# rongmon/rbvfit

Measured on AMD Instinct MI355X. Metric: walker-lnprob evals/sec, higher is better.
Workload: dtype f64; 1 GPU; C1: MgII 2796/2803 z=0.348, 2 components, 4096 px, 23-tap Gaussian LSF; walkers_per_gpu=512, walkers_total=512, ndim=6, n_lines=4, parallelism=walker-shard x1

## Files before the change

rbvfit_amd/csrc/capi_context.inc:

```
namespace {

thread_local std::string g_create_error;
#ifdef VP_STAMPS
double g_host_stamps[8];
std::chrono::steady_clock::time_point g_host_t0;
#define VP_HSTAMP(k) g_host_stamps[k] = std::chrono::duration<double, std::nano>(std::chrono::steady_clock::now() - g_host_t0).count()
#else
#define VP_HSTAMP(k) do { } while (0)
#endif

struct Tuning {
    int prep_rpw = 64;
    int geom = -1;
    int finalize = -1;
    int walker = -1;
    long zerocopy_max = 1l << 20;
    int no_zerocopy = 0;
    int no_multipole = 0;
    int multipole_min = 3;
    int span = 0;
    int waves = 0;
    long lds_pad = 0;
    int no_fused_accept = 0;
    int farfield = -1;
    int no_shared_prep = 0;
    int walker_clusters = 0;
    int multi_sync = 0;
    int host_spin = 2;
    int no_ff_members = 0;
    int tile_multi = -1;
    int gather_plain = 0;
    int tile_lpt = 1;
    int slice_rows = 2;
    int flux_farfield = -1;
    int walker_prio = -1;
    long walker_perm_hex = 0;
    int walker_perm = -1;
    int stretch_overlap = -1;
    int prearm = -1;
    int prearm_us = 500;
    int flux_walker = 1;
    int stretch_mailbox = 1;
    int walker_split = 0;
    int slice_seg = 0;
};

struct Knob { const char* name; const char* env; int is_long; size_t off; };
#define VP_KNOB(field, envname, is_long) {#field, envname, is_long, offsetof(Tuning, field)}
const Knob g_knobs[] = {
    VP_KNOB(prep_rpw, "RBVFIT_AMD_PREP_RPW", 0), VP_KNOB(geom, "RBVFIT_AMD_GEOM", 0),
    VP_KNOB(finalize, "RBVFIT_AMD_FINALIZE", 0), VP_KNOB(walker, "RBVFIT_AMD_WALKER", 0),
    VP_KNOB(zerocopy_max, "RBVFIT_AMD_ZEROCOPY_MAX", 1),
    VP_KNOB(no_zerocopy, "RBVFIT_AMD_NO_ZEROCOPY", 0), VP_KNOB(no_multipole, "RBVFIT_AMD_NO_MULTIPOLE", 0), VP_KNOB(multipole_min, "RBVFIT_AMD_MULTIPOLE_MIN", 0),
    VP_KNOB(span, "RBVFIT_AMD_SPAN", 0), VP_KNOB(waves, "RBVFIT_AMD_WAVES", 0), VP_KNOB(lds_pad, "RBVFIT_AMD_LDS_PAD", 1),
    VP_KNOB(no_fused_accept, "RBVFIT_AMD_NO_FUSED_ACCEPT", 0), VP_KNOB(slice_rows, "RBVFIT_AMD_SLICE_ROWS", 0), VP_KNOB(walker_clusters, "RBVFIT_AMD_WALKER_CLUSTERS", 0), VP_KNOB(no_shared_prep, "RBVFIT_AMD_NO_SHARED_PREP", 0),
    VP_KNOB(farfield, "RBVFIT_AMD_FARFIELD", 0), VP_KNOB(multi_sync, "RBVFIT_AMD_MULTI_SYNC", 0), VP_KNOB(tile_multi, "RBVFIT_AMD_TILE_MULTI", 0), VP_KNOB(no_ff_members, "RBVFIT_AMD_NO_FF_MEMBERS", 0), VP_KNOB(host_spin, "RBVFIT_AMD_HOST_SPIN", 0),
    VP_KNOB(tile_lpt, "RBVFIT_AMD_TILE_LPT", 0), VP_KNOB(gather_plain, "RBVFIT_AMD_GATHER_PLAIN", 0), VP_KNOB(slice_seg, "RBVFIT_AMD_SLICE_SEG", 0),
    VP_KNOB(flux_farfield, "RBVFIT_AMD_FLUX_FARFIELD", 0), VP_KNOB(stretch_overlap, "RBVFIT_AMD_STRETCH_OVERLAP", 0), VP_KNOB(stretch_mailbox, "RBVFIT_AMD_STRETCH_MAILBOX", 0), VP_KNOB(flux_walker, "RBVFIT_AMD_FLUX_WALKER", 0), VP_KNOB(walker_perm, "RBVFIT_AMD_WALKER_PERM", 0), VP_KNOB(walker_prio, "RBVFIT_AMD_WALKER_PRIO", 0), VP_KNOB(walker_perm_hex, "RBVFIT_AMD_WALKER_PERM_HEX", 1),
    VP_KNOB(prearm, "RBVFIT_AMD_PREARM", 0), VP_KNOB(prearm_us, "RBVFIT_AMD_PREARM_US", 0), VP_KNOB(walker_split, "RBVFIT_AMD_WALKER_SPLIT", 0),
};
void set_knob(Tuning& t, const Knob& k, long v) {
    char* base = reinterpret_cast<char*>(&t) + k.off;
    if (k.is_long) *reinterpret_cast<long*>(base) = v; else *reinterpret_cast<int*>(base) = (int)v;
}
Tuning tuning_from_env() {
    Tuning t;
    for (const Knob& k : g_knobs)
        if (const char* e = getenv(k.env))
            set_knob(t, k, *e ? (std::strcmp(k.name, "walker_perm_hex") == 0 ? (long)strtoull(e, nullptr, 16) : strtol(e, nullptr, 10)) : 1);
    return t;
}

struct Instrument {
    vp::InstDev dev{};
    vp::InstDev dev_s{};
    vp::InstDev dev_w{};
    size_t lds_w = 0;
    size_t lds_s = 0;
    int* split_hint = nullptr;
    unsigned long long wperm = 0xFEDCBA9876543210ull;
    unsigned long long wperm_shared = 0xFEDCBA9876543210ull;
    int deal_ntask = 0;
    std::vector<long> deal_cost;

    vp::LinesDev lines{};
    double sum_logw = 0.0;
    std::vector<void*> allocs;
    double* d_flux = nullptr;
    double* d_w = nullptr;
    size_t lds_bytes = 0;
    std::vector<double> h_lambda0, h_gamma;
    std::vector<int> h_bidx;
    bool needs_generic = true;
    bool nanfix = false;
    int nwaves = 1;
    bool ff_on = false;
    double ff_cover = 0.0;
    int ff_items = 0;
    std::vector<double> h_lines;
    std::vector<int> h_idx;
    unsigned long long member_mask[2] = {0ull, 0ull};
    bool same_lines_as_prev = false;
    int* fisher_off = nullptr;
    int2* fisher_terms = nullptr;
// ... 130 lines not shown
int fail(const vp_ctx* c, int code, const std::string& msg) {
    if (c) c->err = msg; else g_create_error = msg;
    return code;
}

#define HIP_TRY(c, expr)                                                                     \
    do {                                                                                     \
        hipError_t e__ = (expr);                                                             \
        if (e__ != hipSuccess)                                                               \
            return fail((c), VP_EHIP, std::string(#expr) + ": " + hipGetErrorString(e__));   \
    } while (0)

template <class T>
int upload(vp_ctx* c, Instrument* ins, const T* host, size_t n, T** out, size_t pad = 0) {
    T* d = nullptr;
    HIP_TRY(c, hipMalloc((void**)&d, ((n ? n : 1) + pad) * sizeof(T)));
    if (ins) ins->allocs.push_back(d);
    if (pad) HIP_TRY(c, hipMemset(d + n, 0, pad * sizeof(T)));
    if (n) HIP_TRY(c, hipMemcpy(d, host, n * sizeof(T), hipMemcpyHostToDevice));
    *out = d;
    return VP_OK;
}

double neumaier_sum(const double* v, int n) {
    double s = 0.0, comp = 0.0;
    for (int i = 0; i < n; ++i) {
        double t = s + v[i];
        if (std::fabs(s) >= std::fabs(v[i])) comp += (s - t) + v[i]; else comp += (v[i] - t) + s;
        s = t;
    }
    return s + comp;
}

constexpr uint64_t VP_SENTINEL_BITS = 0x7FF8A5C3965A3C69ull;
inline bool carries_sentinel(const double* v, size_t n) {
    bool hit = false;
    for (size_t i = 0; i < n; ++i) {
        uint64_t b;
        std::memcpy(&b, v + i, 8);
        hit |= ((b & 0x7FFFFFFFFFFFFFFFull) | 0x0008000000000000ull) == VP_SENTINEL_BITS;
    }
    return hit;
}

int ensure_scratch(vp_ctx* c, size_t bytes) {
    if (bytes <= c->scratch_bytes) return VP_OK;
// ... 93 lines not shown
```

rbvfit_amd/csrc/capi_launch.inc:

```
struct TileOpts {
    const vp::InstDev* geom = nullptr;
    int grid_z = 1;
    double* ff = nullptr;
    int gen_slots = 0;
    const double* theta_rebuild = nullptr;
    int D = 0;
};
template <int OUT, bool GENERIC>
void launch_tile(const Instrument& in, const double* lc, const int* flags, double* out, int stride, int offset,
                 int W, hipStream_t s, const vp::FinalizeArgs& fin, const int* genflag, const TileOpts& o = TileOpts{}) {
    const vp::InstDev& dev = o.geom ? *o.geom : in.dev;
    const bool fast = dev.method == VP_VOIGT_FAST;
    dim3 grid(W, dev.ntiles, o.grid_z);
    dim3 block(64 * in.nwaves);
    const dim3 gg(o.gen_slots > 0 ? std::min(W, o.gen_slots) : W, dev.ntiles, o.grid_z);
    if (dev.rbot && OUT != 2) {
        constexpr int O = OUT == 1 ? 1 : 0;
        if (GENERIC)
            hipLaunchKernelGGL((vp::tile_generic_kernel<O, false, true>), gg, block, in.lds_bytes, s, dev, lc, flags, out, stride, offset, fin, genflag, W,
                               in.lines, (const double*)nullptr, 0);
        else
            hipLaunchKernelGGL((fast ? vp::tile_kernel<1, O, false, false, true> : vp::tile_kernel<0, O, false, false, true>), grid, block, in.lds_bytes, s,
                               dev, lc, flags, out, stride, offset, fin, genflag);
        return;
// ... 190 lines not shown
        if (c->inst.size() == 2)
            hipLaunchKernelGGL((fast ? vp::walker_kernel2<1, SAMPLER, ARMED> : vp::walker_kernel2<0, SAMPLER, ARMED>), grid, block, lds, s, dk[0], dk[1], tb, t0, a, st);
        else
            hipLaunchKernelGGL((fast ? vp::walker_kernel4<1, SAMPLER, ARMED> : vp::walker_kernel4<0, SAMPLER, ARMED>), grid, block, lds, s, dk[0], dk[1], dk[2], dk[3],
                               tb, t0, a, st);
        return;
    }
    hipLaunchKernelGGL((fast ? vp::walker_kernel<1, false, SAMPLER, ARMED> : keep_clusters ? vp::walker_kernel<0, true, false, ARMED>
                                                                                            : vp::walker_kernel<0, false, SAMPLER, ARMED>),
                       grid, block, lds, s, d0, t0, a, st);
}

unsigned long long walker_deal_for(vp_ctx* c, int W, bool shared_ok) {
    const unsigned long long ident = 0xFEDCBA9876543210ull;
    const int mode = c->tune.walker_perm;
    if (c->inst.size() != 1 || mode == 0) return ident;
    if (c->tune.walker_perm_hex != 0) return (unsigned long long)c->tune.walker_perm_hex;
    const Instrument& in = c->inst[0];
    if (mode == 1) return in.wperm;
    if (mode == 2 && shared_ok) return in.wperm_shared;
    if (ctx_num_cus(c) > 0 && W <= ctx_num_cus(c)) return in.wperm;
    return shared_ok ? in.wperm_shared : ident;
}
int walker_prio_for(vp_ctx* c, int W) {
    if (c->tune.walker_prio >= 0) return c->tune.walker_prio ? 1 : 0;
    return (ctx_num_cus(c) > 0 && W <= ctx_num_cus(c)) ? 0 : 1;
}

vp::WalkerArgs walker_args(vp_ctx* c, int W, const double* theta, double* out, double sum_logw, int split = 0, int row0 = 0,
                           bool shared_cus = false, bool shared_ok = false) {
    const Instrument& in = c->inst[0];
    const size_t nrec = (size_t)(in.dev.L + in.dev.NCm) * vp::LC_STRIDE;
    const int per = std::max(1, split);
    vp::WalkerArgs a{theta, c->d_lb, c->d_ub, c->d_lc + (size_t)row0 * per * nrec, out, sum_logw, c->D,
                     (int)((split > 0 ? in.lds_s : walker_wave_lds(c)) / sizeof(double)),
                     (shared_cus && c->tune.walker_prio < 0) ? 1 : walker_prio_for(c, W * per),
                     split > 0 ? 0xFEDCBA9876543210ull : walker_deal_for(c, W, shared_ok)};
    if (split > 0) { a.split = split; a.split_row0 = row0; a.split_part = c->d_partial; a.split_ticket = c->d_ticket; }
    return a;
}

struct LaunchPlan {
    int kind = 0;
    int split = 0;
    int Wp = 0;
    int sel = 0;
    int fmode = 0;
    int ff_first = -1;
    int ff_first_blk = 0;
};
const vp::InstDev& geom_of(const Instrument& x, int sel) { return sel == 2 ? x.dev_w : sel ? x.dev_s : x.dev; }

void launch_walker(vp_ctx* c, const LaunchPlan& p, int W, const double* d_theta, double* d_out, hipStream_t s, bool armed = false) {
    vp::WalkerArgs a = walker_args(c, W, d_theta, d_out, c->inst[0].sum_logw, p.split, 0, false, !armed);
    if (armed) {
        a.arm_slots = c->arm.slots;
        a.arm_slot_doubles = c->arm.slot_doubles;
        a.arm_host = c->arm.h_dev;
        a.arm_seq = c->arm.seq;
        const int cap = std::min(std::max(1, c->tune.prearm_us), 100000);
// ... 213 lines not shown
```

rbvfit_amd/csrc/capi_misc.inc:

```
void vp_philox4x32(const uint32_t ctr[4], const uint32_t key[2], uint32_t out[4]) {
    const vp::Philox4 r = vp::philox4x32_10(ctr[0], ctr[1], ctr[2], ctr[3], key[0], key[1]);
    for (int i = 0; i < 4; ++i) out[i] = r.v[i];
}

int vp_voigt_h(vp_ctx* c, int na, const double* a, int nx, const double* x, double* out) {
    if (!c) return VP_EINVAL;
    CtxGuard g(c);
    if (na <= 0 || nx <= 0 || !a || !x || !out) return fail(c, VP_EINVAL, "vp_voigt_h: empty or NULL input");
    HIP_TRY(c, hipSetDevice(c->device));
    const size_t rec = (size_t)na * vp::LC_STRIDE, need = (rec + na + nx + (size_t)na * nx) * sizeof(double);
    int rc;
    if ((rc = ensure_scratch(c, need))) return rc;
    double* d_rec = c->d_scratch;
    double* d_a = d_rec + rec;
    double* d_x = d_a + na;
    double* d_o = d_x + nx;
    HIP_TRY(c, hipMemcpyAsync(d_a, a, na * sizeof(double), hipMemcpyHostToDevice, c->stream));
    HIP_TRY(c, hipMemcpyAsync(d_x, x, nx * sizeof(double), hipMemcpyHostToDevice, c->stream));
    hipLaunchKernelGGL(vp::prep_h_kernel, dim3((na + 63) / 64), dim3(64), 0, c->stream, d_a, (int)na, d_rec);
    hipLaunchKernelGGL(vp::voigt_h_kernel, dim3((nx + 255) / 256, na), dim3(256), 0, c->stream, d_rec, d_x, nx, d_o);
    HIP_TRY(c, hipGetLastError());
    HIP_TRY(c, hipMemcpyAsync(out, d_o, (size_t)na * nx * sizeof(double), hipMemcpyDeviceToHost, c->stream));
    HIP_TRY(c, hipStreamSynchronize(c->stream));
    return VP_OK;
// ... 58 lines not shown
    if (pairs) *pairs = 0;
    const vp_ctx::LastFF lf = c->last_ff;
    if (lf.inst < 0 || !lf.ff || lf.W <= 0 || lf.nbk <= 0) return VP_OK;
    HIP_TRY(c, hipSetDevice(c->device));
    HIP_TRY(c, hipDeviceSynchronize());
    const size_t n = (size_t)lf.W * lf.nbk;
    std::vector<double> h(n * vp::FF_STRIDE);
    HIP_TRY(c, hipMemcpy(h.data(), lf.ff, h.size() * sizeof(double), hipMemcpyDeviceToHost));
    const Instrument& in = c->inst[lf.inst];
    int64_t cov = 0, mem = 0;
    for (size_t i = 0; i < n; ++i) {
        unsigned long long m[2];
        memcpy(m, h.data() + i * vp::FF_STRIDE + vp::FF_MASK0, sizeof m);
        cov += __builtin_popcountll(m[0]) + __builtin_popcountll(m[1]);
        mem += __builtin_popcountll(m[0] & in.member_mask[0]) + __builtin_popcountll(m[1] & in.member_mask[1]);
    }
    if (variant) *variant = lf.members ? 2 : 1;
    if (covered) *covered = cov;
    if (covered_members) *covered_members = mem;
    if (pairs) *pairs = (int64_t)n * in.lines.L;
    return VP_OK;
}

int vp_walker_deals(const vp_ctx* c, int inst, uint64_t deals[2], int64_t* cost, int max_tiles, int* ntiles, int* ntask) {
    if (!c) return VP_EINVAL;
    std::lock_guard<std::mutex> g(c->mu);
    if (inst < 0 || inst >= (int)c->inst.size()) return VP_EINVAL;
    const Instrument& in = c->inst[inst];
    if (deals) { deals[0] = in.wperm; deals[1] = in.wperm_shared; }
    if (ntiles) *ntiles = in.dev_w.ntiles;
    if (ntask) *ntask = in.deal_ntask;
    for (int t = 0; cost && t < max_tiles; ++t) cost[t] = t < (int)in.deal_cost.size() ? in.deal_cost[t] : 0;
    return VP_OK;
}
int vp_last_launch_kind(const vp_ctx* c) {
    if (!c) return -1;
    std::lock_guard<std::mutex> g(c->mu);
    return c->last_kind;
}
int vp_last_walker_split(const vp_ctx* c) {
    if (!c) return -1;
    std::lock_guard<std::mutex> g(c->mu);
    return c->last_kind == 1 ? c->last_split : 0;
}
```

rbvfit_amd/csrc/capi_setup.inc:

```

const char* vp_version(void) { return "rbvfit_amd " RBVFIT_AMD_VERSION " (gfx950, hip)"; }

int vp_device_count(void) {
    int n = 0;
    if (hipGetDeviceCount(&n) != hipSuccess) return 0;
    return n;
}

const char* vp_last_error(const vp_ctx* ctx) { return ctx ? ctx->err.c_str() : g_create_error.c_str(); }

int vp_ctx_create(vp_ctx** out, int device_id) {
    if (!out) return fail(nullptr, VP_EINVAL, "out is NULL");
    *out = nullptr;
    int n = 0;
    hipError_t e = hipGetDeviceCount(&n);
    if (e != hipSuccess || n <= 0)
        return fail(nullptr, VP_EHIP, std::string("no usable HIP device: ") + (e != hipSuccess ? hipGetErrorString(e) : "device count is 0"));
    if (device_id < 0 || device_id >= n) return fail(nullptr, VP_EINVAL, "device_id out of range");
    vp_ctx* c = new (std::nothrow) vp_ctx();
    if (!c) return fail(nullptr, VP_ENOMEM, "out of host memory");
    c->device = device_id;
    c->tune = tuning_from_env();
    if ((e = hipSetDevice(device_id)) != hipSuccess || (e = hipStreamCreateWithFlags(&c->stream, hipStreamNonBlocking)) != hipSuccess) {
        std::string m = std::string("context creation failed: ") + hipGetErrorString(e);
// ... 148 lines not shown
        Kuse = K; cidx = K / 2;
        double norm = 1.0;
        if (lsf_mode == VP_LSF_ASTROPY_EXTEND) { norm = 0.0; for (int j = 0; j < K; ++j) norm += taps[j]; }
        kflip.resize(K);
        for (int j = 0; j < K; ++j) {
            double t = taps[K - 1 - j];
            kflip[j] = (lsf_mode == VP_LSF_ASTROPY_EXTEND) ? t / norm : t;
        }
    }
    std::vector<double> ginv(P);
    for (int p = 0; p < P; ++p) ginv[p] = 1.0 / wave[p];
    double *d_wave, *d_ginv, *d_flux, *d_w, *d_k, *d_l0, *d_g, *d_f, *d_z, *d_fr0;
    std::vector<double> freq0(L);
    for (int l = 0; l < L; ++l) freq0[l] = vp::C_FREQ / lambda0[l];
    int *d_n, *d_b, *d_v;
#define UP(T, h, n, d) if ((rc = upload<T>(c, &in, h, n, &d))) { for (void* p : in.allocs) hipFree(p); return rc; }
    UP(double, wave, P, d_wave) UP(double, ginv.data(), P, d_ginv)
    if ((rc = upload<double>(c, &in, flux, P, &d_flux, vp::OBS_PAD)) || (rc = upload<double>(c, &in, inv_sigma2, P, &d_w, vp::OBS_PAD))) {
        for (void* p : in.allocs) hipFree(p);
        return rc;
    }
    kflip.resize((kflip.size() + 7) & ~(size_t)7, 0.0);
    UP(double, kflip.data(), kflip.size(), d_k)
    UP(double, lambda0, L, d_l0) UP(double, freq0.data(), L, d_fr0) UP(double, gamma, L, d_g) UP(double, f, L, d_f) UP(double, zfac, L, d_z)
    UP(int, N_idx, L, d_n) UP(int, b_idx, L, d_b) UP(int, v_idx, L, d_v)
    in.d_flux = d_flux; in.d_w = d_w;
    std::vector<int> cl_mp(L, -1), cl_end(L, 0), cl_first, cl_count;
    for (int l = 0; l < L;) {
        int e = l + 1;
        while (e < L && lambda0[e] == lambda0[l] && zfac[e] == zfac[l]) ++e;
        for (int k = l; k < e; ++k) cl_end[k] = e;
        const bool enable = !c->tune.no_multipole;
        if (enable && e - l >= c->tune.multipole_min && e - l <= 64 && voigt_method == VP_VOIGT_WOFZ) {
            cl_mp[l] = (int)cl_first.size();
            cl_first.push_back(l);
            cl_count.push_back(e - l);
        }
        l = e;
    }
    const int NCm = (int)cl_first.size();
    for (int k = 0; k < NCm; ++k)
        for (int l = cl_first[k]; l < cl_first[k] + cl_count[k] && l < 128; ++l) in.member_mask[l >> 6] |= 1ull << (l & 63);
    int *d_clmp, *d_clend, *d_clfirst, *d_clcount;
    UP(int, cl_mp.data(), L, d_clmp) UP(int, cl_end.data(), L, d_clend)
    UP(int, cl_first.data(), cl_first.size(), d_clfirst) UP(int, cl_count.data(), cl_count.size(), d_clcount)
    std::vector<int4> mem_info;
    for (int k = 0; k < NCm; ++k) {
        const int m0 = (int)mem_info.size();
// ... 186 lines not shown
                unsigned long long perm = 0xFEDCBA9876543210ull;
                for (int k = 0; k < nw; ++k) {
                    const int tier = k / 4, lo = tier * 4, hi = std::min(nw, lo + 4) - 1;
                    const int tile = idx[(tier & 1) ? hi - (k - lo) : k];
                    perm = (perm & ~(15ull << (4 * seq[k]))) | ((unsigned long long)tile << (4 * seq[k]));
                }
                in.wperm = perm;
                {
                    long cmax = 0;
                    for (int t = 0; t < nw; ++t) cmax = std::max(cmax, cost[t]);
                    std::vector<int> asc(nw);
                    for (int t = 0; t < nw; ++t) asc[t] = t;
                    std::stable_sort(asc.begin(), asc.end(), [&](int a, int b) { return cost[a] < cost[b]; });
                    std::vector<int> grp(nw, 2);
                    for (int t = 0; t < nw; ++t) if (cmax > 0 && 2 * cost[t] > cmax) grp[t] = 1;
                    for (int k = 0; k < ntask; ++k) grp[asc[k]] = 0;
                    unsigned long long ps = 0xFEDCBA9876543210ull;
                    int k = 0;
                    for (int g = 0; g < 3; ++g)
                        for (int t = 0; t < nw; ++t)
                            if (grp[t] == g) { ps = (ps & ~(15ull << (4 * k))) | ((unsigned long long)t << (4 * k)); ++k; }
                    in.wperm_shared = ps;
                }
                in.deal_ntask = ntask;
                in.deal_cost.assign(cost.begin(), cost.end());
            }
            int* d_tabl;
            if ((rc = upload<int>(c, &in, tabl.data(), tabl.size(), &d_tabl))) { for (void* p : in.allocs) hipFree(p); return rc; }
            gd->core_hint = d_tabl;
        }
    }
    in.h_lambda0.assign(lambda0, lambda0 + L); in.h_gamma.assign(gamma, gamma + L); in.h_bidx.assign(b_idx, b_idx + L);
    in.h_lines.assign(lambda0, lambda0 + L); in.h_lines.insert(in.h_lines.end(), gamma, gamma + L);
    in.h_lines.insert(in.h_lines.end(), f, f + L); in.h_lines.insert(in.h_lines.end(), zfac, zfac + L);
    in.h_idx.assign(N_idx, N_idx + L); in.h_idx.insert(in.h_idx.end(), b_idx, b_idx + L); in.h_idx.insert(in.h_idx.end(), v_idx, v_idx + L);
    in.h_idx.push_back(voigt_method); in.h_idx.push_back(c->tune.no_multipole); in.h_idx.push_back(c->tune.multipole_min);
    if (!c->inst.empty()) {
        const Instrument& pv = c->inst.back();
        in.same_lines_as_prev = pv.h_idx == in.h_idx && pv.h_lines.size() == in.h_lines.size() &&
                                std::memcmp(pv.h_lines.data(), in.h_lines.data(), in.h_lines.size() * sizeof(double)) == 0;
    }
    analyse_generic(c, in);
    if (c->tune.lds_pad > 0) in.lds_bytes += (size_t)c->tune.lds_pad;
    c->inst.push_back(std::move(in));
    c->meta_dirty = true;
    if (inst_index) *inst_index = (int)c->inst.size() - 1;
// ... 33 lines not shown
```

rbvfit_amd/csrc/voigt_kernels.h:

```cpp
#pragma once
#include "voigt_device.h"
#include "sampler_kernels.h"

namespace vp {

#ifndef VP_DIAG
#define VP_DIAG 0
#endif
enum { ABL_NOFAR = 1,
       ABL_NONEAR = 2,
       ABL_NOCORE = 4,
       ABL_NOEXP = 8,
       ABL_NOLSF = 16,
       ABL_NOCHI = 32,
       ABL_ENTRY = 64,
       ABL_NOSMALLEXP = 128,
       ABL_NOPRIO = 256,
       ABL_EMPTY = 512,
       ABL_NOFFPOLY = 1024,
       ABL_NOMP = 2048 };
#define VP_ABL(bit) ((VP_DIAG & (bit)) != 0)

struct LinesDev {
    int L;
// ... 123 lines not shown
            const double hn2 = hn * hn;
            const double tb = exp(-hn2) / (hn2 + a2);
            S1 += tb;
            rec[LC_TBL0 + n] = (0.5 * ALG916_C * a) * tb;
        }
    }
    const double pref = T * (a * INV_SQRT_PI);
#pragma unroll
    for (int m = 0; m < NWING; ++m) {
        double cm = 0.0;
#pragma unroll
        for (int i = m; i >= 0; --i) cm = __builtin_fma(cm, a2, g_wing.c[m][i]);
        rec[LC_K0 + m] = pref * cm;
    }
    rec[LC_T] = T;
    rec[LC_Y] = a;
    rec[LC_ACOS] = (mode == 1) ? erfcx(a) - (ALG916_C * a) * S1 : 0.0;
    reinterpret_cast<int*>(rec + LC_MODE)[0] = mode;
    reinterpret_cast<int*>(rec + LC_MODE)[1] = core_terms(a);
    rec[LC_EA2] = (mode == 0) ? 1.0 + a2 * (1.0 + a2 * (0.5 + a2 * (1.0 / 6 + a2 * (1.0 / 24)))) : exp(a2);
}

struct LineScalars { double d, freq0, ibf, a, Tl, cfd, Ax, Bx; };
__device__ __forceinline__ LineScalars line_scalars_nbv(double thN, double b, double v, const LinesDev& T, int l) {
    LineScalars s;
    const double lam0 = T.lambda0[l], gam = T.gamma[l], fo = T.f[l], zf = T.zfac[l];
    const double N = exp10(thN);
    const double z_total = zf * (1.0 + v / C_KMS) - 1.0;
    s.d = 1.0 + z_total;
    const double b_f = b / lam0 * 1e13;
    s.freq0 = T.freq0[l];
    s.ibf = fast_rcp(b_f);
    const double constant = ATOMIC_CONSTANT * fast_rcp(s.freq0 * b);
    s.a = gam * (s.ibf * 0.079577471545947667884);
    s.Tl = (N * fo) * constant;
    s.cfd = C_FREQ * s.d;
    s.Ax = s.cfd * s.ibf;
    s.Bx = s.freq0 * s.ibf;
    return s;
}
__device__ __forceinline__ LineScalars line_scalars(const double* __restrict__ th, const LinesDev& T, int l) {
    return line_scalars_nbv(th[T.N_idx[l]], th[T.b_idx[l]], th[T.v_idx[l]], T, l);
}

__device__ __forceinline__ void prep_cluster(const double* __restrict__ th, const LinesDev& T, int k,
                                             double* __restrict__ rec) {
    const int first = T.cl_first[k], n = T.cl_count[k];
    bool allok = true;
    double Ac = 1.79e308, g0sum = 0.0;
    for (int j = 0; j < n; ++j) {
        const LineScalars s = line_scalars(th, T, first + j);
        allok = allok && (s.a >= 0.0) && (s.a <= 0.1) && (fabs(s.Tl) <= 1.79e308) && (fabs(s.Ax) <= 1.79e308)
                && (fabs(s.Bx) <= 1.79e308) && (s.Ax > 0.0);
        Ac = fmin(Ac, s.Ax);
        g0sum += s.Bx * fast_rcp(s.Ax);
    }
    const double g0c = g0sum / (double)n;
    const double Bc = Ac * g0c;
    double dmax = 0.0;
    double Q[MP_NQ];
#pragma unroll
    for (int jq = 0; jq < MP_NQ; ++jq) Q[jq] = 0.0;
    for (int j = 0; j < n; ++j) {
        const LineScalars s = line_scalars(th, T, first + j);
        const double g0 = s.Bx * fast_rcp(s.Ax);
// ... 1220 lines not shown
    }
}

struct TileMulti { int t[3]; int off[4]; };
template <int METHOD>
__global__ __launch_bounds__(64, VP_TILE_WPE) void tile_kernel_multi(InstDev I0, InstDev I1, InstDev I2, InstDev I3, TileMulti tb, int ninst,
                                                                     const double* __restrict__ lc, const int* __restrict__ flags,
                                                                     double* __restrict__ out, int out_stride, FinalizeArgs F) {
    extern __shared__ double fl[];
    const int t = blockIdx.y, w = blockIdx.x;
    const int ki = (ninst > 1 && t >= tb.t[0]) ? ((ninst > 2 && t >= tb.t[1]) ? ((ninst > 3 && t >= tb.t[2]) ? 3 : 2) : 1) : 0;
    const InstDev& I = ki == 0 ? I0 : (ki == 1 ? I1 : (ki == 2 ? I2 : I3));
    const int lt = ki == 0 ? t : t - tb.t[ki - 1];
    const int oob = flags[w];
    const int p0 = lt * I.TP, nout = min(p0 + I.TP, I.P) - p0;
    const TilePre pre = tile_preload(I, p0, nout, threadIdx.x);
    if (oob) return;
    rec_t lcw = as_rec(lc + (size_t)w * (I.L + I.NCm) * LC_STRIDE);
    const double wsum = wave_sum(tile_work<METHOD, 0, false, false>(I, lcw, fl, p0, nout, w, threadIdx.x, 64, pre, true, out, out_stride VP_STAMP_NONE,
                                                                   false, lt));
    if (threadIdx.x == 0) publish_partial(F, out, out_stride, w, tb.off[ki] + lt, wsum);
}

__device__ __forceinline__ void prep_record_lanes(double thv, const LinesDev& T, int l0, double* __restrict__ lcw, int lane) {
    const int j = lane >> 4, slot = lane & 15, l = min(l0 + j, T.L - 1);
    double wc[NWING];
#pragma unroll
    for (int i = 0; i < NWING; ++i) wc[i] = g_wing.c[min(slot, NWING - 1)][i];
    const int iN = T.N_idx[l], ib = T.b_idx[l], iv = T.v_idx[l];
    const LineScalars s = line_scalars_nbv(__shfl(thv, iN, 64), __shfl(thv, ib, 64), __shfl(thv, iv, 64), T, l);
    if (l0 + j >= T.L) return;
    const bool xok = (fabs(s.Ax) <= 1.79e308) && (fabs(s.Bx) <= 1.79e308);
    const double Tl = xok ? s.Tl : __builtin_nan(""), a = s.a;
    double* __restrict__ rec = lcw + (size_t)l * LC_STRIDE;
    if (slot < NWING) {
        const double a2 = a * a;
        const double pref = Tl * (a * INV_SQRT_PI);
        double cm = 0.0;
#pragma unroll
        for (int i = NWING - 1; i >= 0; --i)
            cm = (i <= slot) ? __builtin_fma(cm, a2, wc[i]) : cm;
        rec[LC_K0 + slot] = pref * cm;
    } else if (slot == 14) {
        rec[LC_A] = s.Ax;
        rec[LC_B] = s.Bx;
        rec[LC_D] = s.d;
        rec[LC_RD] = 1.0 / s.d;
        rec[LC_CFD] = s.cfd;
        rec[LC_FREQ0] = s.freq0;
        rec[LC_IBF] = s.ibf;
    } else {
        int mode = 0;
        if (!(a >= 0.0) || !(a < 7.0)) mode = 2;
// ... 20 lines not shown
    double* chain_lp;
    double a;
    uint64_t seed, step;
    int s0, c0, nC, half;
    Replicas rep;
    int ovl, need, mine;
    int* ver;
    const double* pos_c; const double* pos_x; double* pos_w;
    const double* lp_x; double* lp_w;
    int* timeout;
};

struct WalkerArgs {
    const double* theta;
    const double* lb;
    const double* ub;
    double* lc;
    double* lnprob;
    double sum_logw;
    int D;
    int wave_lds;
    int prio;
    unsigned long long wperm;
    const double* arm_slots;
    unsigned int* arm_host;
    unsigned int arm_seq;
    int arm_ticks;
    int arm_slot_doubles;
    int flux_stride;
    int* genflag;
    int* genflag_clear;
    int* gen_any;
    int* gen_any_clear;
    int split;
    int split_row0;
    double* split_part;
    unsigned int* split_ticket;
};

constexpr int ARM_GO = 1, ARM_LEAVE = 2;
constexpr int ARM_EXPIRED_WORD = 16, ARM_STUCK_WORD = 32;
__device__ __forceinline__ int arm_wait(const WalkerArgs& A, int w, int wid, int lane, double& thv, bool first_group, int nslots) {
    const int n = A.arm_slot_doubles;
    const unsigned long long* slot = reinterpret_cast<const unsigned long long*>(A.arm_slots) + (size_t)w * n;
    const bool keeper = first_group && wid == 0;
    const long long t0 = keeper ? wall_clock64() : 0ll;
// ... 41 lines not shown
        } else if (spins > SYNC_SPIN_LIMIT) {
            if (lane == 0) __hip_atomic_store(A.arm_host + ARM_STUCK_WORD, A.arm_seq, __ATOMIC_RELAXED, __HIP_MEMORY_SCOPE_SYSTEM);
            return ARM_LEAVE;
        }
        __builtin_amdgcn_s_sleep(2);
    }
}

__device__ __forceinline__ void walker_result(const WalkerArgs& A, const Replicas& R, int w, double lnp) {
    if (A.lnprob) A.lnprob[w] = lnp;
    if (R.n > 0) {
        for (int r = 0; r < R.n; ++r) {
            if (r == R.me) R.lp[r][w] = lnp;
            else __hip_atomic_store(R.lp[r] + w, lnp, __ATOMIC_RELAXED, __HIP_MEMORY_SCOPE_SYSTEM);
        }
    }
}

struct WalkerMore { int t[3]; double slw[3]; };
template <int METHOD, bool CLUSTERS, bool SAMPLER, int NI, bool ARMED = false, int FLUX = 0, bool SPLIT = false>
#ifndef VP_WALKER_WPE
#define VP_WALKER_WPE 6
#endif
__device__ __forceinline__ void walker_body(InstDev I0, InstDev I1, InstDev I2, InstDev I3, WalkerMore tb, LinesDev T, WalkerArgs A, StretchArgs S) {
    extern __shared__ double smem[];
    if (VP_ABL(ABL_EMPTY)) { if (threadIdx.x == 0 && A.lnprob) A.lnprob[blockIdx.x] = 0.0; return; }
    VP_STAMP_DECL
    VP_STAMP(0);
#ifdef VP_STAMPS
    const long long rt_entry = wall_clock64();
    long long rt_go = rt_entry;
#endif
#ifdef VP_STAMPS
    {
        unsigned int hwid, xcc;
        asm volatile("s_getreg_b32 %0, hwreg(HW_REG_HW_ID)" : "=s"(hwid));
        asm volatile("s_getreg_b32 %0, hwreg(HW_REG_XCC_ID)" : "=s"(xcc));
        if (g_stamp_w >= 0 && g_stamp_w < STAMP_W && (threadIdx.x & 63) == 0)
            g_stamps[(g_stamp_w * STAMP_WAVES + (int)(threadIdx.x >> 6)) * STAMP_STAGES + 7] = (long long)hwid | ((long long)xcc << 32);
    }
#endif
    const int wb = blockIdx.x;
    const int w = SPLIT ? wb / A.split : wb, sg = SPLIT ? wb - w * A.split : 0;
    const int tid = threadIdx.x, lane = tid & 63, nw = blockDim.x >> 6;
    const int wid = __builtin_amdgcn_readfirstlane(tid >> 6);
    double* __restrict__ fl = smem + (size_t)wid * A.wave_lds;
    double* __restrict__ red = smem + (size_t)nw * A.wave_lds;
    const int nrec = T.L + T.NCm;
    double* __restrict__ lcw = A.lc + (size_t)wb * nrec * LC_STRIDE;
    double thv;
    int arm_code = ARM_GO;
    double* __restrict__ stash = red + nw + 2;
    if (SAMPLER) {
        replicas_wait(S.rep);
        const Philox4 r = draw(S.seed, S.step, S.half, S.s0 + w, 0u);
        const double t = (S.a - 1.0) * u01(r.v[0], r.v[1]) + 1.0;
        const double z = t * t / S.a;
        int j = (int)(u01(r.v[2], r.v[3]) * (double)S.nC);
        j = j < S.nC - 1 ? j : S.nC - 1;
        const int d = min(lane, A.D - 1);
        const double* __restrict__ posX = S.ovl ? S.pos_x : S.pos;
        const double* __restrict__ lpX = S.ovl ? S.lp_x : S.lp;
        double x = 0.0, c = 0.0;
        const bool uses_theta = !S.ovl || wid < 1 + ((T.L + 3) >> 2) + (CLUSTERS ? ((T.NCm + 63) >> 6) : 0) || wid == nw - 1;
        if (uses_theta && S.ovl == 2) {
            x = posX[(size_t)(S.s0 + w) * 8 + d];
            const unsigned long long* line = reinterpret_cast<const unsigned long long*>(S.pos_c) + (size_t)(S.c0 + j) * 8;
            for (int spins = 0;; ++spins) {
                const unsigned long long v = __hip_atomic_load(line + (lane == 63 ? 7 : d), __ATOMIC_RELAXED, __HIP_MEMORY_SCOPE_AGENT);
                if ((int)__builtin_amdgcn_readlane((unsigned int)v, 63) >= S.need) {
                    c = __longlong_as_double((long long)v);
                    const unsigned int lo = __builtin_amdgcn_readlane((unsigned int)v, 62), hi = __builtin_amdgcn_readlane((unsigned int)(v >> 32), 62);
                    if (lane == 63) c = __longlong_as_double((long long)(lo | ((unsigned long long)hi << 32)));
                    break;
// ... 10 lines not shown
                int spins = 0;
                while (__hip_atomic_load(S.ver + S.c0 + j, __ATOMIC_RELAXED, __HIP_MEMORY_SCOPE_AGENT) < S.need) {
                    if (++spins > SYNC_SPIN_LIMIT) {
                        if (lane == 0) __hip_atomic_store(S.timeout, 1, __ATOMIC_RELAXED, __HIP_MEMORY_SCOPE_AGENT);
                        break;
                    }
                    __builtin_amdgcn_s_sleep(2);
                }
                c = __hip_atomic_load(S.pos_c + (size_t)(S.c0 + j) * A.D + d, __ATOMIC_RELAXED, __HIP_MEMORY_SCOPE_AGENT);
            } else {
                c = S.pos[(size_t)(S.c0 + j) * A.D + d];
            }
        }
        thv = c - (c - x) * z;
        if (wid == nw - 1) {
            const double lp_old = S.ovl == 2 ? posX[(size_t)(S.s0 + w) * 8 + 6] : lpX[S.s0 + w];
            const Philox4 r1 = draw(S.seed, S.step, S.half, S.s0 + w, 1u);
            const double lz = (double)(A.D - 1) * log(z), lu = log(u01(r1.v[0], r1.v[1]));
            if (lane == 0) { stash[0] = lz; stash[1] = lu; stash[2] = lp_old; }
            stash[4 + lane] = x;
            stash[68 + lane] = thv;
        }
    } else {
        if (ARMED) thv = 0.0;
        else
        thv = A.theta[(size_t)w * A.D + min(lane, A.D - 1)];
        if (S.rep.n > 0) replicas_handshake(S.rep);
    }
#ifdef VP_STAMPS
    VP_STAMP(8);
    asm volatile("s_waitcnt vmcnt(0)" :: "v"(thv) : "memory");
    VP_STAMP(9);
#endif
    const int tw_all = SPLIT ? sg * nw + wid : (int)((A.wperm >> (4 * wid)) & 15ull);
    const bool has_tile = !SPLIT || tw_all < I0.ntiles;
    const int tw = SPLIT ? min(tw_all, I0.ntiles - 1) : tw_all;
    const int ki = (NI > 1 && tw >= tb.t[0]) ? ((NI > 2 && tw >= tb.t[1]) ? ((NI > 3 && tw >= tb.t[2]) ? 3 : 2) : 1) : 0;
    const InstDev& I = ki == 0 ? I0 : (ki == 1 ? I1 : (ki == 2 ? I2 : I3));
    const int lt = ki == 0 ? tw : tw - tb.t[ki - 1];
    const int p0 = lt * I.TP, nout = min(p0 + I.TP, I.P) - p0;
    const int hint_v = METHOD == 0 ? I.core_hint[lt] : 0;
    const int ngrp = (T.L + 3) >> 2, ncl = CLUSTERS ? ((T.NCm + 63) >> 6) : 0;
    const int ntask = 1 + ngrp + ncl;
    auto run_tasks = [&](double th, bool rehearsal) {
        for (int task = wid; task < ntask; task += nw) {
            if (task == 0) {
                if (FLUX) {
                    if (lane == 0) {
                        red[nw] = 0.0;
                        if (A.genflag_clear) A.genflag_clear[w] = 0;
                        if (A.gen_any_clear && w == 0) *A.gen_any_clear = 0;
                    }
                } else {
                const bool oob = lane < A.D && ((th < A.lb[min(lane, A.D - 1)]) || (th > A.ub[min(lane, A.D - 1)]));
                const bool any = __ballot(oob) != 0ull;
                if (lane == 0) red[nw] = any ? 1.0 : 0.0;
                }
            } else if (task <= ngrp) {
                prep_record_lanes(th, T, (task - 1) * 4, lcw, lane);
            } else if (CLUSTERS && !rehearsal) {
                const int k = (task - 1 - ngrp) * 64 + lane;
                const double* trow = ARMED ? A.arm_slots + (size_t)w * A.arm_slot_doubles : A.theta + (size_t)w * A.D;
                if (k < T.NCm) prep_cluster(trow, T, k, lcw + (size_t)(T.L + k) * LC_STRIDE);
            }
        }
    };
    TilePre pre;
    bool daw_ready;
    if (ARMED) {
        if (lane < EXP_LDS_DOUBLES) fl[I.span + FL_PAD + 4 + DAW_LDS_DOUBLES + lane] = exp2_eighth(lane);
        daw_ready = METHOD == 0 && __builtin_amdgcn_readfirstlane(hint_v) != 0;
        if (daw_ready) dawson_to_lds(fl + I.span + FL_PAD + 4, lane, 64);
        if (wid < ntask) {
#pragma nounroll
            for (int pass = 0; pass < 2; ++pass) {
                if (pass == 0) {
                    const int dl = min(lane, A.D - 1);
                    thv = 0.5 * (A.lb[dl] + A.ub[dl]);
                } else {
                    arm_code = arm_wait(A, w, wid, lane, thv, wb == 0, SPLIT ? (int)gridDim.x / A.split : (int)gridDim.x);
#ifdef VP_STAMPS
                    rt_go = wall_clock64();
#endif
                    if (arm_code != ARM_GO) break;
                }
                run_tasks(thv, pass == 0);
            }
            if (lane == 0) stash[wid] = arm_code == ARM_GO ? 1.0 : 2.0;
            asm volatile("s_waitcnt vmcnt(0)" ::: "memory");
        }
        VP_STAMP(10);
        pre = tile_preload(I, p0, nout, lane);
    } else {
        run_tasks(thv, false);
        VP_STAMP(10);
        if (wid < ntask) asm volatile("s_waitcnt vmcnt(0)" ::: "memory");
        pre = tile_preload(I, p0, nout, lane);
        if (lane < EXP_LDS_DOUBLES) fl[I.span + FL_PAD + 4 + DAW_LDS_DOUBLES + lane] = exp2_eighth(lane);
        daw_ready = METHOD == 0 && __builtin_amdgcn_readfirstlane(hint_v) != 0;
        if (daw_ready) dawson_to_lds(fl + I.span + FL_PAD + 4, lane, 64);
    }
    VP_STAMP(11);
    __syncthreads();
    VP_STAMP(1);
#ifdef VP_STAMPS
    if ((!ARMED || arm_code == ARM_GO) && lane == 0 && w < STAMP_W) {
        long long* gs = g_stamps + (w * STAMP_WAVES + wid) * STAMP_STAGES;
        gs[14] = rt_entry; gs[12] = rt_go; gs[13] = wall_clock64();
    }
#endif
    if (!VP_ABL(ABL_NOPRIO) && daw_ready && A.prio) __builtin_amdgcn_s_setprio(VP_PRIO_LEVEL);
    if (ARMED) {
        bool leave = false;
        for (int k = 0; k < min(ntask, nw); ++k) leave = leave || stash[k] != 1.0;
        if (leave) return;
    }
    const bool oobw = red[nw] != 0.0;
    if (VP_ABL(ABL_ENTRY) && !SAMPLER && !FLUX) { if (tid == 0) walker_result(A, S.rep, w, 0.0); return; }
    if (oobw && !SAMPLER) {
        if (tid == 0 && sg == 0) walker_result(A, S.rep, w, -__builtin_inf());
        return;
    }
// ... 180 lines not shown
```

Measured before the change: 24.56 million evals/s.

## Hoist line constants and bounds loads to kernel entry, precompute core-hint mask

Line tables are padded to a multiple of four so each prep wave can load its group's constants through scalar (constant address space) loads at kernel entry, overlapping them with the theta load. Bound checks preload lb/ub early, and the task loop is restructured so wave 0 does the bounds check after the record tasks. A host-computed per-tile core mask replaces the per-block core_hint global load when deciding whether to stage the Dawson table. This is meant to shorten the dependent-load latency chain at walker kernel entry, in exchange for more code complexity and extra registers held across entry.

Result: slower. 23.54 million evals/s (-4.2%).

```diff
diff --git a/rbvfit_amd/csrc/capi_context.inc b/rbvfit_amd/csrc/capi_context.inc
--- a/rbvfit_amd/csrc/capi_context.inc
+++ b/rbvfit_amd/csrc/capi_context.inc
@@ -35,6 +35,7 @@
     int flux_farfield = -1;
     int walker_prio = -1;
     long walker_perm_hex = 0;
+    int walker_core_mask = -1;
     int walker_perm = -1;
     int stretch_overlap = -1;
     int prearm = -1;
@@ -56,7 +57,7 @@
     VP_KNOB(no_fused_accept, "RBVFIT_AMD_NO_FUSED_ACCEPT", 0), VP_KNOB(slice_rows, "RBVFIT_AMD_SLICE_ROWS", 0), VP_KNOB(walker_clusters, "RBVFIT_AMD_WALKER_CLUSTERS", 0), VP_KNOB(no_shared_prep, "RBVFIT_AMD_NO_SHARED_PREP", 0),
     VP_KNOB(farfield, "RBVFIT_AMD_FARFIELD", 0), VP_KNOB(multi_sync, "RBVFIT_AMD_MULTI_SYNC", 0), VP_KNOB(tile_multi, "RBVFIT_AMD_TILE_MULTI", 0), VP_KNOB(no_ff_members, "RBVFIT_AMD_NO_FF_MEMBERS", 0), VP_KNOB(host_spin, "RBVFIT_AMD_HOST_SPIN", 0),
     VP_KNOB(tile_lpt, "RBVFIT_AMD_TILE_LPT", 0), VP_KNOB(gather_plain, "RBVFIT_AMD_GATHER_PLAIN", 0), VP_KNOB(slice_seg, "RBVFIT_AMD_SLICE_SEG", 0),
-    VP_KNOB(flux_farfield, "RBVFIT_AMD_FLUX_FARFIELD", 0), VP_KNOB(stretch_overlap, "RBVFIT_AMD_STRETCH_OVERLAP", 0), VP_KNOB(stretch_mailbox, "RBVFIT_AMD_STRETCH_MAILBOX", 0), VP_KNOB(flux_walker, "RBVFIT_AMD_FLUX_WALKER", 0), VP_KNOB(walker_perm, "RBVFIT_AMD_WALKER_PERM", 0), VP_KNOB(walker_prio, "RBVFIT_AMD_WALKER_PRIO", 0), VP_KNOB(walker_perm_hex, "RBVFIT_AMD_WALKER_PERM_HEX", 1),
+    VP_KNOB(flux_farfield, "RBVFIT_AMD_FLUX_FARFIELD", 0), VP_KNOB(stretch_overlap, "RBVFIT_AMD_STRETCH_OVERLAP", 0), VP_KNOB(stretch_mailbox, "RBVFIT_AMD_STRETCH_MAILBOX", 0), VP_KNOB(flux_walker, "RBVFIT_AMD_FLUX_WALKER", 0), VP_KNOB(walker_perm, "RBVFIT_AMD_WALKER_PERM", 0), VP_KNOB(walker_prio, "RBVFIT_AMD_WALKER_PRIO", 0), VP_KNOB(walker_perm_hex, "RBVFIT_AMD_WALKER_PERM_HEX", 1), VP_KNOB(walker_core_mask, "RBVFIT_AMD_WALKER_CORE_MASK", 0),
     VP_KNOB(prearm, "RBVFIT_AMD_PREARM", 0), VP_KNOB(prearm_us, "RBVFIT_AMD_PREARM_US", 0), VP_KNOB(walker_split, "RBVFIT_AMD_WALKER_SPLIT", 0),
 };
 void set_knob(Tuning& t, const Knob& k, long v) {
@@ -80,6 +81,7 @@
     int* split_hint = nullptr;
     unsigned long long wperm = 0xFEDCBA9876543210ull;
     unsigned long long wperm_shared = 0xFEDCBA9876543210ull;
+    unsigned int core_mask = 0u;
     int deal_ntask = 0;
     std::vector<long> deal_cost;
 
@@ -256,6 +258,14 @@
     return VP_OK;
 }
 
+inline size_t padded_lines(int L) { return ((size_t)L + 3) & ~(size_t)3; }
+template <class T>
+std::vector<T> pad_line_table(const T* host, int L) {
+    std::vector<T> v(host, host + L);
+    v.resize(padded_lines(L), host[L - 1]);
+    return v;
+}
+
 double neumaier_sum(const double* v, int n) {
     double s = 0.0, comp = 0.0;
     for (int i = 0; i < n; ++i) {
diff --git a/rbvfit_amd/csrc/capi_launch.inc b/rbvfit_amd/csrc/capi_launch.inc
--- a/rbvfit_amd/csrc/capi_launch.inc
+++ b/rbvfit_amd/csrc/capi_launch.inc
@@ -236,6 +236,16 @@
     if (ctx_num_cus(c) > 0 && W <= ctx_num_cus(c)) return in.wperm;
     return shared_ok ? in.wperm_shared : ident;
 }
+unsigned int walker_core_mask_for(const vp_ctx* c) {
+    if (c->tune.walker_core_mask >= 0) return (unsigned int)c->tune.walker_core_mask & 0xFFFFu;
+    unsigned int m = 0u;
+    int t0 = 0;
+    for (const Instrument& in : c->inst) {
+        if (t0 < 16) m |= (in.core_mask << t0) & 0xFFFFu;
+        t0 += in.dev_w.ntiles;
+    }
+    return m;
+}
 int walker_prio_for(vp_ctx* c, int W) {
     if (c->tune.walker_prio >= 0) return c->tune.walker_prio ? 1 : 0;
     return (ctx_num_cus(c) > 0 && W <= ctx_num_cus(c)) ? 0 : 1;
@@ -249,7 +259,8 @@
     vp::WalkerArgs a{theta, c->d_lb, c->d_ub, c->d_lc + (size_t)row0 * per * nrec, out, sum_logw, c->D,
                      (int)((split > 0 ? in.lds_s : walker_wave_lds(c)) / sizeof(double)),
                      (shared_cus && c->tune.walker_prio < 0) ? 1 : walker_prio_for(c, W * per),
-                     split > 0 ? 0xFEDCBA9876543210ull : walker_deal_for(c, W, shared_ok)};
+                     split > 0 ? 0xFEDCBA9876543210ull : walker_deal_for(c, W, shared_ok),
+                     split > 0 ? 0u : walker_core_mask_for(c)};
     if (split > 0) { a.split = split; a.split_row0 = row0; a.split_part = c->d_partial; a.split_ticket = c->d_ticket; }
     return a;
 }
diff --git a/rbvfit_amd/csrc/capi_misc.inc b/rbvfit_amd/csrc/capi_misc.inc
--- a/rbvfit_amd/csrc/capi_misc.inc
+++ b/rbvfit_amd/csrc/capi_misc.inc
@@ -104,6 +104,12 @@
     return VP_OK;
 }
 
+int vp_test_pad_line_table(const double* table, int L, double* out, int cap) {
+    if (!table || L <= 0 || !out) return -1;
+    const std::vector<double> v = pad_line_table(table, L);
+    for (int i = 0; i < (int)v.size() && i < cap; ++i) out[i] = v[i];
+    return (int)v.size();
+}
 int vp_walker_deals(const vp_ctx* c, int inst, uint64_t deals[2], int64_t* cost, int max_tiles, int* ntiles, int* ntask) {
     if (!c) return VP_EINVAL;
     std::lock_guard<std::mutex> g(c->mu);
diff --git a/rbvfit_amd/csrc/capi_setup.inc b/rbvfit_amd/csrc/capi_setup.inc
--- a/rbvfit_amd/csrc/capi_setup.inc
+++ b/rbvfit_amd/csrc/capi_setup.inc
@@ -194,8 +194,11 @@
     }
     kflip.resize((kflip.size() + 7) & ~(size_t)7, 0.0);
     UP(double, kflip.data(), kflip.size(), d_k)
-    UP(double, lambda0, L, d_l0) UP(double, freq0.data(), L, d_fr0) UP(double, gamma, L, d_g) UP(double, f, L, d_f) UP(double, zfac, L, d_z)
-    UP(int, N_idx, L, d_n) UP(int, b_idx, L, d_b) UP(int, v_idx, L, d_v)
+    UP(double, pad_line_table(lambda0, L).data(), padded_lines(L), d_l0) UP(double, pad_line_table(freq0.data(), L).data(), padded_lines(L), d_fr0)
+    UP(double, pad_line_table(gamma, L).data(), padded_lines(L), d_g) UP(double, pad_line_table(f, L).data(), padded_lines(L), d_f)
+    UP(double, pad_line_table(zfac, L).data(), padded_lines(L), d_z)
+    UP(int, pad_line_table(N_idx, L).data(), padded_lines(L), d_n) UP(int, pad_line_table(b_idx, L).data(), padded_lines(L), d_b)
+    UP(int, pad_line_table(v_idx, L).data(), padded_lines(L), d_v)
     in.d_flux = d_flux; in.d_w = d_w;
     std::vector<int> cl_mp(L, -1), cl_end(L, 0), cl_first, cl_count;
     for (int l = 0; l < L;) {
@@ -428,6 +431,8 @@
                             if (grp[t] == g) { ps = (ps & ~(15ull << (4 * k))) | ((unsigned long long)t << (4 * k)); ++k; }
                     in.wperm_shared = ps;
                 }
+                in.core_mask = 0u;
+                for (int t = 0; t < nw; ++t) if (cost[t] > 0) in.core_mask |= 1u << t;
                 in.deal_ntask = ntask;
                 in.deal_cost.assign(cost.begin(), cost.end());
             }
diff --git a/rbvfit_amd/csrc/voigt_kernels.h b/rbvfit_amd/csrc/voigt_kernels.h
--- a/rbvfit_amd/csrc/voigt_kernels.h
+++ b/rbvfit_amd/csrc/voigt_kernels.h
@@ -169,14 +169,18 @@
 }
 
 struct LineScalars { double d, freq0, ibf, a, Tl, cfd, Ax, Bx; };
-__device__ __forceinline__ LineScalars line_scalars_nbv(double thN, double b, double v, const LinesDev& T, int l) {
+struct LineConsts { double lambda0, gamma, f, zfac, freq0; };
+__device__ __forceinline__ LineConsts line_consts(const LinesDev& T, int l) {
+    return LineConsts{T.lambda0[l], T.gamma[l], T.f[l], T.zfac[l], T.freq0[l]};
+}
+__device__ __forceinline__ LineScalars line_scalars_nbv(double thN, double b, double v, const LineConsts& K) {
     LineScalars s;
-    const double lam0 = T.lambda0[l], gam = T.gamma[l], fo = T.f[l], zf = T.zfac[l];
+    const double lam0 = K.lambda0, gam = K.gamma, fo = K.f, zf = K.zfac;
     const double N = exp10(thN);
     const double z_total = zf * (1.0 + v / C_KMS) - 1.0;
     s.d = 1.0 + z_total;
     const double b_f = b / lam0 * 1e13;
-    s.freq0 = T.freq0[l];
+    s.freq0 = K.freq0;
     s.ibf = fast_rcp(b_f);
     const double constant = ATOMIC_CONSTANT * fast_rcp(s.freq0 * b);
     s.a = gam * (s.ibf * 0.079577471545947667884);
@@ -187,7 +191,7 @@
     return s;
 }
 __device__ __forceinline__ LineScalars line_scalars(const double* __restrict__ th, const LinesDev& T, int l) {
-    return line_scalars_nbv(th[T.N_idx[l]], th[T.b_idx[l]], th[T.v_idx[l]], T, l);
+    return line_scalars_nbv(th[T.N_idx[l]], th[T.b_idx[l]], th[T.v_idx[l]], line_consts(T, l));
 }
 
 __device__ __forceinline__ void prep_cluster(const double* __restrict__ th, const LinesDev& T, int k,
@@ -1454,13 +1458,34 @@
     if (threadIdx.x == 0) publish_partial(F, out, out_stride, w, tb.off[ki] + lt, wsum);
 }
 
-__device__ __forceinline__ void prep_record_lanes(double thv, const LinesDev& T, int l0, double* __restrict__ lcw, int lane) {
+typedef const int __attribute__((address_space(4)))* irec_t;
+struct GroupConsts { double lambda0[4], gamma[4], f[4], zfac[4], freq0[4]; int N_idx[4], b_idx[4], v_idx[4]; };
+struct LaneLine { LineConsts k; int iN, ib, iv; };
+__device__ __forceinline__ GroupConsts load_group_consts(const LinesDev& T, int l0) {
+    GroupConsts g;
+    const rec_t pl = (rec_t)reinterpret_cast<unsigned long long>(T.lambda0 + l0), pg = (rec_t)reinterpret_cast<unsigned long long>(T.gamma + l0),
+                pf = (rec_t)reinterpret_cast<unsigned long long>(T.f + l0), pz = (rec_t)reinterpret_cast<unsigned long long>(T.zfac + l0),
+                pq = (rec_t)reinterpret_cast<unsigned long long>(T.freq0 + l0);
+    const irec_t pN = (irec_t)reinterpret_cast<unsigned long long>(T.N_idx + l0), pb = (irec_t)reinterpret_cast<unsigned long long>(T.b_idx + l0),
+                 pv = (irec_t)reinterpret_cast<unsigned long long>(T.v_idx + l0);
+#pragma unroll
+    for (int j = 0; j < 4; ++j) {
+        g.lambda0[j] = pl[j]; g.gamma[j] = pg[j]; g.f[j] = pf[j]; g.zfac[j] = pz[j]; g.freq0[j] = pq[j];
+        g.N_idx[j] = pN[j]; g.b_idx[j] = pb[j]; g.v_idx[j] = pv[j];
+    }
+    return g;
+}
+__device__ __forceinline__ LaneLine pick_lane_line(const GroupConsts& g, int lane) {
+    const int j = lane >> 4;
+    auto sel = [j](const auto (&a)[4]) { return j == 0 ? a[0] : j == 1 ? a[1] : j == 2 ? a[2] : a[3]; };
+    return LaneLine{LineConsts{sel(g.lambda0), sel(g.gamma), sel(g.f), sel(g.zfac), sel(g.freq0)}, sel(g.N_idx), sel(g.b_idx), sel(g.v_idx)};
+}
+__device__ __forceinline__ void prep_record_lanes(double thv, const LinesDev& T, const LaneLine& q, int l0, double* __restrict__ lcw, int lane) {
     const int j = lane >> 4, slot = lane & 15, l = min(l0 + j, T.L - 1);
     double wc[NWING];
 #pragma unroll
     for (int i = 0; i < NWING; ++i) wc[i] = g_wing.c[min(slot, NWING - 1)][i];
-    const int iN = T.N_idx[l], ib = T.b_idx[l], iv = T.v_idx[l];
-    const LineScalars s = line_scalars_nbv(__shfl(thv, iN, 64), __shfl(thv, ib, 64), __shfl(thv, iv, 64), T, l);
+    const LineScalars s = line_scalars_nbv(__shfl(thv, q.iN, 64), __shfl(thv, q.ib, 64), __shfl(thv, q.iv, 64), q.k);
     if (l0 + j >= T.L) return;
     const bool xok = (fabs(s.Ax) <= 1.79e308) && (fabs(s.Bx) <= 1.79e308);
     const double Tl = xok ? s.Tl : __builtin_nan(""), a = s.a;
@@ -1527,6 +1552,7 @@
     int wave_lds;
     int prio;
     unsigned long long wperm;
+    unsigned int core_mask;
     const double* arm_slots;
     unsigned int* arm_host;
     unsigned int arm_seq;
@@ -1614,6 +1640,18 @@
 #ifndef VP_WALKER_WPE
 #define VP_WALKER_WPE 6
 #endif
+#ifndef VP_ENTRY_P1
+#define VP_ENTRY_P1 1
+#endif
+#ifndef VP_ENTRY_P2
+#define VP_ENTRY_P2 1
+#endif
+#ifndef VP_ENTRY_P3
+#define VP_ENTRY_P3 1
+#endif
+#ifndef VP_ENTRY_P4
+#define VP_ENTRY_P4 1
+#endif
 __device__ __forceinline__ void walker_body(InstDev I0, InstDev I1, InstDev I2, InstDev I3, WalkerMore tb, LinesDev T, WalkerArgs A, StretchArgs S) {
     extern __shared__ double smem[];
     if (VP_ABL(ABL_EMPTY)) { if (threadIdx.x == 0 && A.lnprob) A.lnprob[blockIdx.x] = 0.0; return; }
@@ -1642,6 +1680,12 @@
     double* __restrict__ lcw = A.lc + (size_t)wb * nrec * LC_STRIDE;
     double thv;
     int arm_code = ARM_GO;
+    const int ngrp = (T.L + 3) >> 2, ncl = CLUSTERS ? ((T.NCm + 63) >> 6) : 0;
+    const int ntask = 1 + ngrp + ncl;
+    constexpr bool EARLY_CONSTS = VP_ENTRY_P1 && !SAMPLER && !ARMED;
+    const bool rec_wave = wid >= 1 && wid <= ngrp;
+    LaneLine q0{};
+    double lbv = 0.0, ubv = 0.0;
     double* __restrict__ stash = red + nw + 2;
     if (SAMPLER) {
         replicas_wait(S.rep);
@@ -1698,9 +1742,19 @@
             stash[68 + lane] = thv;
         }
     } else {
-        if (ARMED) thv = 0.0;
-        else
-        thv = A.theta[(size_t)w * A.D + min(lane, A.D - 1)];
+        thv = 0.0;
+        if (EARLY_CONSTS && rec_wave) {
+            const GroupConsts gc = load_group_consts(T, (wid - 1) * 4);
+            thv = A.theta[(size_t)w * A.D + min(lane, A.D - 1)];
+            asm volatile("" ::: "memory");
+            q0 = pick_lane_line(gc, lane);
+        } else
+        if (!ARMED && (!VP_ENTRY_P4 || wid < ntask)) thv = A.theta[(size_t)w * A.D + min(lane, A.D - 1)];
+        if (VP_ENTRY_P2 && !ARMED && !FLUX && wid == 0) {
+            lbv = A.lb[min(lane, A.D - 1)];
+            ubv = A.ub[min(lane, A.D - 1)];
+        }
+        asm volatile("" ::: "memory");
         if (S.rep.n > 0) replicas_handshake(S.rep);
     }
 #ifdef VP_STAMPS
@@ -1715,29 +1769,34 @@
     const InstDev& I = ki == 0 ? I0 : (ki == 1 ? I1 : (ki == 2 ? I2 : I3));
     const int lt = ki == 0 ? tw : tw - tb.t[ki - 1];
     const int p0 = lt * I.TP, nout = min(p0 + I.TP, I.P) - p0;
-    const int hint_v = METHOD == 0 ? I.core_hint[lt] : 0;
-    const int ngrp = (T.L + 3) >> 2, ncl = CLUSTERS ? ((T.NCm + 63) >> 6) : 0;
-    const int ntask = 1 + ngrp + ncl;
+    const bool core_masked = VP_ENTRY_P3 && METHOD == 0 && !SPLIT && ((A.core_mask >> tw_all) & 1u) != 0u;
+    int hint_v = 0;
+    if (METHOD == 0 && !core_masked) hint_v = I.core_hint[lt];
     auto run_tasks = [&](double th, bool rehearsal) {
-        for (int task = wid; task < ntask; task += nw) {
-            if (task == 0) {
-                if (FLUX) {
-                    if (lane == 0) {
-                        red[nw] = 0.0;
-                        if (A.genflag_clear) A.genflag_clear[w] = 0;
-                        if (A.gen_any_clear && w == 0) *A.gen_any_clear = 0;
-                    }
-                } else {
-                const bool oob = lane < A.D && ((th < A.lb[min(lane, A.D - 1)]) || (th > A.ub[min(lane, A.D - 1)]));
-                const bool any = __ballot(oob) != 0ull;
-                if (lane == 0) red[nw] = any ? 1.0 : 0.0;
-                }
-            } else if (task <= ngrp) {
-                prep_record_lanes(th, T, (task - 1) * 4, lcw, lane);
+        for (int task = wid == 0 ? nw : wid; task < ntask; task += nw) {
+            if (task <= ngrp) {
+                LaneLine q = q0;
+                if (!EARLY_CONSTS || task != wid) q = pick_lane_line(load_group_consts(T, (task - 1) * 4), lane);
+                prep_record_lanes(th, T, q, (task - 1) * 4, lcw, lane);
             } else if (CLUSTERS && !rehearsal) {
                 const int k = (task - 1 - ngrp) * 64 + lane;
                 const double* trow = ARMED ? A.arm_slots + (size_t)w * A.arm_slot_doubles : A.theta + (size_t)w * A.D;
                 if (k < T.NCm) prep_cluster(trow, T, k, lcw + (size_t)(T.L + k) * LC_STRIDE);
+            }
+        }
+        if (wid == 0) {
+            if (FLUX) {
+                if (lane == 0) {
+                    red[nw] = 0.0;
+                    if (A.genflag_clear) A.genflag_clear[w] = 0;
+                    if (A.gen_any_clear && w == 0) *A.gen_any_clear = 0;
+                }
+            } else {
+                const bool early = VP_ENTRY_P2 && !ARMED && !SAMPLER;
+                const double lo = early ? lbv : A.lb[min(lane, A.D - 1)], hi = early ? ubv : A.ub[min(lane, A.D - 1)];
+                const bool oob = lane < A.D && ((th < lo) || (th > hi));
+                const bool any = __ballot(oob) != 0ull;
+                if (lane == 0) red[nw] = any ? 1.0 : 0.0;
             }
         }
     };
@@ -1745,7 +1804,7 @@
     bool daw_ready;
     if (ARMED) {
         if (lane < EXP_LDS_DOUBLES) fl[I.span + FL_PAD + 4 + DAW_LDS_DOUBLES + lane] = exp2_eighth(lane);
-        daw_ready = METHOD == 0 && __builtin_amdgcn_readfirstlane(hint_v) != 0;
+        daw_ready = core_masked || (METHOD == 0 && __builtin_amdgcn_readfirstlane(hint_v) != 0);
         if (daw_ready) dawson_to_lds(fl + I.span + FL_PAD + 4, lane, 64);
         if (wid < ntask) {
 #pragma nounroll
@@ -1773,7 +1832,7 @@
         if (wid < ntask) asm volatile("s_waitcnt vmcnt(0)" ::: "memory");
         pre = tile_preload(I, p0, nout, lane);
         if (lane < EXP_LDS_DOUBLES) fl[I.span + FL_PAD + 4 + DAW_LDS_DOUBLES + lane] = exp2_eighth(lane);
-        daw_ready = METHOD == 0 && __builtin_amdgcn_readfirstlane(hint_v) != 0;
+        daw_ready = core_masked || (METHOD == 0 && __builtin_amdgcn_readfirstlane(hint_v) != 0);
         if (daw_ready) dawson_to_lds(fl + I.span + FL_PAD + 4, lane, 64);
     }
     VP_STAMP(11);
```
